# lizhiqi49/threestudio-3dgs

Hardware: AMD Instinct MI355X
Metric: rendered views/sec fwd+bwd @1M Gaussians, 1024², SH=3; 1/2/4/8 GPU (higher is better)
Workload: dtype fp32

## Files before the change

include/gsr.h:

```cpp
#ifndef GSR_H
#define GSR_H

#include <stddef.h>
#include <stdint.h>

#ifdef __cplusplus
extern "C" {
#endif

#define GSR_OK 0
#define GSR_EINVAL 1
#define GSR_EHIP 2

#define GSR_TILE_X 16
#define GSR_TILE_Y 16

const char* gsr_version(void);
#define GSR_ABI_VERSION 9
int gsr_abi_version(void);
const char* gsr_last_error(void);

size_t gsr_geom_bytes(int P);
size_t gsr_binning_bytes(int K, int width, int height);
size_t gsr_image_bytes(int width, int height);
// ... 285 lines not shown
int gsr_sugar_deform_forward(const gsr_sugar_deform* in, float* xyz, float* rot, float* scale, void* stream);
int gsr_sugar_deform_backward(const gsr_sugar_deform* in, const int* sp_order, const int* sp_offsets,
                              const int* col_order, const int* col_offsets, const int* t_order, const int* t_offsets,
                              const float* dL_dxyz, const float* dL_drot, const float* dL_dscale,
                              float* const* dL_dplanes, float* const* dL_dmlp, void* workspace, size_t workspace_bytes,
                              void* stream);

#define GSR_MESHREG_FORWARD 0
#define GSR_MESHREG_NC_BACKWARD 1
#define GSR_MESHREG_LAP_BACKWARD 2
typedef struct gsr_sugar_meshreg {
  int T, V, E, P;
  const float* vert_xyz;
  const int* pairs;
  const int* slot_offsets;
  const int* slots;
  const int* ring_offsets;
  const int* ring;
} gsr_sugar_meshreg;
size_t gsr_sugar_meshreg_workspace_bytes(int T, int V, int P, int pass);
int gsr_sugar_normal_consistency_forward(const gsr_sugar_meshreg* in, float* nc, void* workspace,
                                         size_t workspace_bytes, void* stream);
int gsr_sugar_normal_consistency_backward(const gsr_sugar_meshreg* in, const float* dL_dnc, float* dL_dvert_xyz,
                                          void* workspace, size_t workspace_bytes, void* stream);
int gsr_sugar_laplacian_forward(const gsr_sugar_meshreg* in, float* lap, void* workspace, size_t workspace_bytes,
                                void* stream);
int gsr_sugar_laplacian_backward(const gsr_sugar_meshreg* in, const float* dL_dlap, float* dL_dvert_xyz,
                                 void* workspace, size_t workspace_bytes, void* stream);

size_t gsr_sort_work_bytes(int V, const int* n);
int gsr_sort_pairs(int V, const int* n, uint32_t* keys, uint32_t* vals, int key_bits, int max_bits, void* work,
                   size_t work_bytes, void* stream);
int gsr_sort_rank_mode(void);

int gsr_mark_visible(int P, const float* means3D, const float* viewmatrix, const float* projmatrix,
                     uint8_t* present, void* stream);

#ifdef __cplusplus
}
#endif

#endif
```

threestudio-3dgs_amd/csrc/gsr_api.hip:

```cpp
#include <stdio.h>
#include <string.h>

#include <cmath>
#include <mutex>
#include <vector>

#include "../../include/gsr.h"
#include "gsr_kernels.h"

using namespace gsr;

static thread_local char g_err[512] = "";

static int fail(int code, const char* fmt, const char* what) {
  snprintf(g_err, sizeof(g_err), fmt, what);
  return code;
}

#define GSR_HIP_CHECK(expr)                                                        \
  do {                                                                             \
    hipError_t e_ = (expr);                                                        \
    if (e_ != hipSuccess) return fail(GSR_EHIP, "HIP error: %s", hipGetErrorString(e_)); \
  } while (0)

// ... 213 lines not shown
  hipStream_t s = (hipStream_t)stream;
  GeomState g = GeomState::carve(state->geom, V, P, nullptr);

  PreprocessArgs a;
  a.V = V;
  a.P = P;
  a.deg = effective_degree(sc.degree, sc.M);
  a.M = sc.M;
  a.means3D = sc.means3D;
  a.scales = sc.scales;
  a.rotations = sc.rotations;
  a.opacities = sc.opacities;
  a.shs = sc.shs;
  a.colors_precomp = sc.colors_precomp;
  a.cov3D_precomp = sc.cov3D_precomp;
  a.scale_modifier = sc.scale_modifier;
  a.W = sc.width;
  a.H = sc.height;
  a.radii = state->radii;
  a.col2 = colors2;
  {
    PhaseScope ps(GSR_PHASE_PREPROCESS, s);
    launch_preprocess(a, cams, g, s);
  }
  {
    PhaseScope ps(GSR_PHASE_DEPTH_SORT, s);
    SegInfo seg;
    seg.V = V;
    for (int v = 0; v < V; ++v) {
      seg.n[v] = (uint32_t)P;
      seg.start[v] = (uint32_t)((size_t)v * P);
    }
    seg.rebase = g.drange + 128;
    const int res = seg_sort(g.dkey, g.dval, false, seg, 0, 32, g.sort_counts, g.sort_totals, s);
    if (res != depth_sort_result()) return fail(GSR_EHIP, "%s", "internal: depth sort result buffer");
    launch_binning_counts(V, P, g, s);
  }
  return last_launch();
}

int gsr_composite_forward(int V, int height, int width, const float* color, const float* alpha, const float* bg,
                          int bg_layout, float* out, void* stream) {
  if (V < 0 || height < 0 || width < 0 || bg_layout < 0 || bg_layout > 2) return fail(GSR_EINVAL, "%s", "bad sizes");
  if (V == 0 || height == 0 || width == 0) return last_launch();
  if (color == nullptr || alpha == nullptr || bg == nullptr || out == nullptr)
    return fail(GSR_EINVAL, "%s", "null pointer argument");
  launch_composite_fwd(V, (size_t)height * width, color, alpha, bg, bg_layout, out, (hipStream_t)stream);
  return last_launch();
}

int gsr_composite_backward(int V, int height, int width, const float* dL_dout, const float* color,
                           const float* alpha, const float* bg, int bg_layout, float* dL_dcolor, float* dL_dalpha,
                           float* dL_dbg, void* stream) {
  if (V < 0 || height < 0 || width < 0 || bg_layout < 0 || bg_layout > 2) return fail(GSR_EINVAL, "%s", "bad sizes");
  if (V == 0 || height == 0 || width == 0) return last_launch();
  if (dL_dout == nullptr || color == nullptr || alpha == nullptr || bg == nullptr || dL_dcolor == nullptr ||
      dL_dalpha == nullptr)
    return fail(GSR_EINVAL, "%s", "null pointer argument");
  if (dL_dbg != nullptr && bg_layout == GSR_BG_CONSTANT)
    return fail(GSR_EINVAL, "%s", "dL_dbg is computed for image backgrounds only");
  launch_composite_bwd(V, (size_t)height * width, dL_dout, color, alpha, bg, bg_layout, dL_dcolor, dL_dalpha,
                       dL_dbg, (hipStream_t)stream);
  return last_launch();
}

int gsr_normal_map_forward(int V, int height, int width, const float* normal, const float* alpha, float* out,
                           void* stream) {
// ... 672 lines not shown
  if (!set_total(V, n, seg, &total)) return 0;
  size_t b = 0;
  SortWork::carve(nullptr, V, total, seg.blk[V], &b);
  return b;
}

int gsr_sort_pairs(int V, const int* n, uint32_t* keys, uint32_t* vals, int key_bits, int max_bits, void* work,
                   size_t work_bytes, void* stream) {
  if (V < 1 || V > GSR_SET_MAX) return fail(GSR_EINVAL, "%s", "1..64 segments");
  if (n == nullptr || keys == nullptr || work == nullptr) return fail(GSR_EINVAL, "%s", "null pointer argument");
  if (key_bits < 1 || key_bits > 32 || max_bits < 1 || max_bits > GSR_RADIX_BITS)
    return fail(GSR_EINVAL, "%s", "key_bits must be 1..32 and max_bits 1..8");
  SegInfo seg;
  long long total = 0;
  if (inst_segments(V, n, seg, &total) != GSR_OK) return GSR_EINVAL;
  size_t need = 0;
  SortWork w = SortWork::carve(work, V, total, seg.blk[V], &need);
  if (work_bytes < need) return fail(GSR_EINVAL, "%s", "sort work buffer too small");
  if (total == 0) return last_launch();
  hipStream_t s = (hipStream_t)stream;
  uint32_t* kk[2] = {keys, w.keys2};
  uint32_t* vv[2] = {vals, vals != nullptr ? w.vals2 : nullptr};
  const int r = seg_sort(kk, vals != nullptr ? vv : nullptr, false, seg, 0, key_bits, w.counts, w.totals, s,
                         max_bits);
  if (r == 1) {
    GSR_HIP_CHECK(hipMemcpyAsync(keys, w.keys2, sizeof(uint32_t) * (size_t)total, hipMemcpyDeviceToDevice, s));
    if (vals != nullptr)
      GSR_HIP_CHECK(hipMemcpyAsync(vals, w.vals2, sizeof(uint32_t) * (size_t)total, hipMemcpyDeviceToDevice, s));
  }
  return last_launch();
}

int gsr_sort_rank_mode(void) { return sort_rank_mode(); }

int gsr_set_num_rendered(int V, const void* geom, int P, int* num_rendered, int* num_visible, int* num_listed,
                         void* stream) {
  if (check_set(V, P) != GSR_OK) return GSR_EINVAL;
  if (geom == nullptr || num_rendered == nullptr) return fail(GSR_EINVAL, "%s", "null pointer argument");
  GeomState g = GeomState::carve((void*)geom, V, P, nullptr);
  hipStream_t s = (hipStream_t)stream;
  static thread_local uint32_t* pinned = nullptr;
  if (pinned == nullptr) GSR_HIP_CHECK(hipHostMalloc((void**)&pinned, 3 * GSR_SET_MAX * sizeof(uint32_t), hipHostMallocDefault));
  GSR_HIP_CHECK(hipMemcpyAsync(pinned, g.counters, 3 * (size_t)V * sizeof(uint32_t), hipMemcpyDeviceToHost, s));
  GSR_HIP_CHECK(hipStreamSynchronize(s));
  for (int v = 0; v < V; ++v) {
    num_rendered[v] = (int)pinned[v];
    if (num_visible) num_visible[v] = (int)pinned[V + v];
    if (num_listed) num_listed[v] = (int)pinned[2 * V + v];
    if (pinned[v] > 0x7fffffffu) return fail(GSR_EINVAL, "%s", "instance count of a view exceeds 2^31");
  }
  g_err[0] = 0;
  return GSR_OK;
}

int gsr_set_gauss_state(int V, const void* geom, int P, void* out_rec, void* out_tiles, void* stream) {
  if (check_set(V, P) != GSR_OK) return GSR_EINVAL;
  if (geom == nullptr) return fail(GSR_EINVAL, "%s", "null pointer argument");
  if (P == 0) return GSR_OK;
  GeomState g = GeomState::carve((void*)geom, V, P, nullptr);
  hipStream_t s = (hipStream_t)stream;
  const size_t n = (size_t)V * (size_t)P;
  if (out_rec) GSR_HIP_CHECK(hipMemcpyAsync(out_rec, g.rec, n * sizeof(GaussRec), hipMemcpyDeviceToDevice, s));
  if (out_tiles) GSR_HIP_CHECK(hipMemcpyAsync(out_tiles, g.tiles, n * sizeof(uint2), hipMemcpyDeviceToDevice, s));
  return last_launch();
}

// ... 362 lines not shown
```

threestudio-3dgs_amd/csrc/gsr_common.h:

```cpp
#pragma once

#include <hip/hip_runtime.h>

#if !defined(GSR_DIAG_BUILD) &&                                                                          \
    (defined(GSR_EXP_COALROWS) || defined(GSR_EXP_FWD_NOC) || defined(GSR_EXP_LDSPAD) ||                  \
     defined(GSR_EXP_NOCULL) || defined(GSR_EXP_NOFLUSH) || defined(GSR_EXP_NOGROUP) ||                   \
     defined(GSR_EXP_NOMFMA) || defined(GSR_EXP_NOREACH) || defined(GSR_EXP_NOREPLAY) ||                \
     defined(GSR_EXP_NOCOL2) || defined(GSR_EXP_HOTREC) || defined(GSR_EXP_NOEMBED))
#error "GSR_EXP_* experiment switches build only through `make exp` (a diagnostic library, not libgsr_hip.so)"
#endif
#include <stddef.h>
#include <stdlib.h>
#include <string.h>
#include <stdint.h>

#define GSR_TILE_X 16
#define GSR_TILE_Y 16
#define GSR_TILE_PIX (GSR_TILE_X * GSR_TILE_Y)

#define GSR_SET_MAX 64
#define GSR_SORT_THREADS 256
#ifndef GSR_SORT_ITEMS
#define GSR_SORT_ITEMS 16
#endif
// ... 48 lines not shown
  TilePack t;
  t.tile_bits = tile_key_bits(W, H);
  int gb = 1;
  while (gb < 32 && (1ll << gb) < (long long)P) ++gb;
  t.packed = gb + t.tile_bits <= 32 && !force;
  t.gbits = t.packed ? gb : 0;
  t.gmask = t.packed ? (uint32_t)((1ull << gb) - 1ull) : 0xFFFFFFFFu;
  t.qmask = !t.packed && t.tile_bits <= GSR_QMASK_SHIFT && force_mode != 2;
  t.tmask = t.tile_bits >= 32 ? 0xFFFFFFFFu : (uint32_t)((1ull << t.tile_bits) - 1ull);
  return t;
}

struct DigitPlan {
  int passes, bits;
  __host__ __device__ int width(int p, int key_bits) const {
    const int lo = p * bits;
    return key_bits - lo < bits ? key_bits - lo : bits;
  }
};
static inline DigitPlan digit_plan(int key_bits, int max_bits = GSR_RADIX_BITS) {
  if (key_bits < 1) key_bits = 1;
  if (max_bits < 1 || max_bits > GSR_RADIX_BITS) max_bits = GSR_RADIX_BITS;
  DigitPlan d;
  d.passes = (key_bits + max_bits - 1) / max_bits;
  d.bits = (key_bits + d.passes - 1) / d.passes;
  return d;
}
struct SegInfo {
  int V, tile;
  uint32_t n[GSR_SET_MAX];
  uint32_t start[GSR_SET_MAX];
  uint32_t blk[GSR_SET_MAX + 1];
  const uint32_t* ndev = nullptr;
  const uint32_t* rebase = nullptr;
};
__device__ __forceinline__ uint32_t seg_live(const SegInfo& s, int v) {
  return s.ndev ? min(s.ndev[v], s.n[v]) : s.n[v];
}
__device__ __forceinline__ uint32_t seg_key_base(const SegInfo& s) { return s.rebase ? s.rebase[0] : 0u; }
__device__ __forceinline__ uint32_t seg_key(uint32_t kb, uint32_t key) {
  return key == 0xFFFFFFFFu ? key : key - kb;
}
__device__ __forceinline__ bool seg_skip_last(const SegInfo& s, int last) {
  return last && s.rebase != nullptr && s.rebase[1] != 0u;
}
static inline void seg_fill_blocks(SegInfo& s, int tile) {
  s.tile = tile;
  s.blk[0] = 0;
  for (int v = 0; v < s.V; ++v) s.blk[v + 1] = s.blk[v] + (uint32_t)div_up((long long)s.n[v], tile);
}
__device__ __forceinline__ uint32_t xcd_block(uint32_t b, uint32_t n) {
  const uint32_t x = b & 7u, q = n >> 3, r = n & 7u;
  return x * q + (x < r ? x : r) + (b >> 3);
}
__device__ __forceinline__ int seg_of_block(const SegInfo& s, uint32_t b, uint32_t& lb) {
  int lo = 0, hi = s.V;
  while (hi - lo > 1) {
    const int mid = (lo + hi) >> 1;
    if (s.blk[mid] <= b) lo = mid;
    else hi = mid;
  }
  lb = b - s.blk[lo];
  return lo;
}

struct ViewCam {
  const float *view, *proj, *campos;
  float tanx, tany;
  float fx, fy;
};
struct SetCams {
  ViewCam c[GSR_SET_MAX];
};

struct __attribute__((aligned(64))) GaussRec {
  float4 a, b, c;
  uint4 d;
// ... 10 lines not shown
  uint32_t* goff;
  uint32_t* goff_part;
  uint32_t* vis_part;
  int vbits;
  __host__ __device__ uint32_t vmask() const { return vbits >= 32 ? 0xFFFFFFFFu : (1u << vbits) - 1u; }
  __host__ __device__ uint32_t vsent() const { return vbits > 26 ? 0u : (1u << (32 - vbits)) - 1u; }
  uint32_t* drange;
  __device__ const uint32_t* sorted_dval() const { return drange[129] ? dval[1] : dval[0]; }
  __device__ const uint32_t* sorted_dkey() const { return drange[129] ? dkey[1] : dkey[0]; }
  uint32_t* counters;
  static int sort_blocks(int P) { return div_up(P > 0 ? P : 1, GSR_SORT_TILE); }
  static int dup_blocks(int P) { return div_up(P > 0 ? P : 1, GSR_DUP_TILE); }
  static int goff_blocks(int P) { return div_up(P > 0 ? P : 1, GSR_GOFF_TILE); }
  static GeomState carve(void* base, int V, int P, size_t* bytes) {
    Carver c(base);
    GeomState g;
    const size_t n = (size_t)(V > 0 ? V : 1) * (size_t)(P > 0 ? P : 1);
    const size_t nv = (size_t)(V > 0 ? V : 1);
    g.rec = c.take<GaussRec>(n);
    g.tiles = c.take<uint2>(n);
    g.dkey[0] = c.take<uint32_t>(n);
    g.dkey[1] = c.take<uint32_t>(n);
    g.dval[0] = c.take<uint32_t>(n);
    g.dval[1] = c.take<uint32_t>(n);
    g.sort_counts = c.take<uint32_t>(nv * GSR_RADIX * sort_blocks(P));
    g.sort_totals = c.take<uint32_t>(nv * GSR_RADIX);
    g.kept_counts = c.take<uint32_t>(nv * dup_blocks(P));
    g.counters = c.take<uint32_t>(3 * nv + 64);
    g.goff = c.take<uint32_t>(n);
    g.goff_part = c.take<uint32_t>(nv * goff_blocks(P));
    g.vis_part = c.take<uint32_t>(nv * goff_blocks(P));
    g.vbits = 1;
    while (g.vbits < 32 && (1ull << g.vbits) < (unsigned long long)(P > 1 ? P : 2)) ++g.vbits;
    g.drange = c.take<uint32_t>(132);
    if (bytes) *bytes = align_up(c.off, 256);
    return g;
  }
};

struct BinningState {
  uint32_t* key[2];
  uint32_t* val[2];
  uint32_t* sort_counts;
  uint32_t* sort_totals;
  static BinningState carve(void* base, int V, long long Ktot, long long sort_blocks, bool with_vals, size_t* bytes) {
    Carver c(base);
    BinningState b;
    const size_t n = (size_t)(Ktot > 0 ? Ktot : 1);
    b.key[0] = c.take<uint32_t>(n);
    b.key[1] = c.take<uint32_t>(n);
    b.val[0] = with_vals ? c.take<uint32_t>(n) : nullptr;
    b.val[1] = with_vals ? c.take<uint32_t>(n) : nullptr;
    b.sort_counts = c.take<uint32_t>((size_t)GSR_RADIX * (size_t)(sort_blocks > 0 ? sort_blocks : 1));
    b.sort_totals = c.take<uint32_t>((size_t)GSR_RADIX * (size_t)(V > 0 ? V : 1));
    if (bytes) *bytes = align_up(c.off, 256);
    return b;
  }
};

#define GSR_SPLIT_MAX_TILES 4096
#define GSR_SPLIT_CH 256
#define GSR_SPLIT_NCK 15
__host__ __device__ inline bool split_fits(int V, size_t tiles) {
  return V >= 1 && tiles > 0 && (size_t)V * tiles <= GSR_SPLIT_MAX_TILES;
}
__host__ __device__ inline int split_extra(int V, size_t tiles) {
  const size_t e = (size_t)V * tiles / 4;
// ... 182 lines not shown
```

threestudio-3dgs_amd/csrc/gsr_kernels.h:

```cpp
#pragma once

#include "../../include/gsr.h"
#include "gsr_common.h"

namespace gsr {

int seg_sort(uint32_t* keys[2], uint32_t* vals[2], bool vals_identity, SegInfo seg, int bit_lo, int key_bits,
             uint32_t* counts, uint32_t* totals, hipStream_t stream, int max_bits = GSR_RADIX_BITS);
struct RunWork {
  uint32_t* keys[2];
  uint32_t* vals[2];
  uint32_t *counts, *totals;
  uint32_t* bounds;
  void carve(Carver& c, size_t items, size_t n, float** coef = nullptr) {
    for (int i = 0; i < 2; ++i) keys[i] = c.take<uint32_t>(items);
    for (int i = 0; i < 2; ++i) vals[i] = c.take<uint32_t>(items);
    if (coef) *coef = c.take<float>(items);
    counts = c.take<uint32_t>((size_t)GSR_RADIX * (size_t)div_up((long long)items, GSR_SORT_TILE));
    totals = c.take<uint32_t>((size_t)GSR_RADIX);
    bounds = c.take<uint32_t>(2 * n);
  }
};
int sort_runs(RunWork w, uint32_t n, int N, int* half, hipStream_t stream);
int sort_rank_mode();

struct PreprocessArgs {
  int V, P, deg, M;
  const float *means3D, *scales, *rotations, *opacities, *shs, *colors_precomp, *cov3D_precomp;
  float scale_modifier;
  int W, H;
  int* radii;
  const float* col2;
};
void launch_preprocess(const PreprocessArgs& a, const SetCams& cams, const GeomState& g, hipStream_t stream);

void launch_binning_counts(int V, int P, const GeomState& g, hipStream_t stream);
void launch_emit(int V, int P, int W, const GeomState& g, const SegInfo& inst, const TilePack& tp, uint32_t* keys,
                 uint32_t* vals, hipStream_t stream);
void launch_tile_ranges(SegInfo inst, int n_tiles, const TilePack& tp, const uint32_t* keys, uint2* ranges,
                        hipStream_t stream);
void launch_mark_visible(int P, const float* means3D, const float* view, const float* proj,
                         uint8_t* present, hipStream_t stream);

__device__ __forceinline__ float quad_form(float a, float b, float c, float u, float v) {
  return fmaf(a * u, u, fmaf(2.0f * b * u, v, c * v * v));
}
__device__ __forceinline__ bool quadrant_hit(const float4 r0, const float4 r1, float qx, float qy) {
  const float o = r1.y;
  if (!(o >= GSR_ALPHA_MIN * 0.9999f)) return false;
  const float a = r0.z, b = r0.w, c = r1.x;
  if (!(a > 0.0f && c > 0.0f && a * c - b * b > 0.0f)) return true;
  const float tau = fmaxf(0.0f, __logf(255.0f * o));
  const float thr = 2.0f * (tau * 1.002f + 2e-3f);
  const float u1 = r0.x - qx, u0 = u1 - 7.0f;
  const float v1 = r0.y - qy, v0 = v1 - 7.0f;
  if (u0 <= 0.0f && u1 >= 0.0f && v0 <= 0.0f && v1 >= 0.0f) return true;
  const float ia = 1.0f / a, ic = 1.0f / c;
// ... 180 lines not shown
```

threestudio-3dgs_amd/csrc/gsr_preprocess.hip:

```cpp
#include "gsr_kernels.h"
#include "gsr_math.h"

namespace gsr {

void launch_preprocess_kernel(const PreprocessArgs& a, const SetCams& cams, const GeomState& g, hipStream_t stream);

#ifndef GSR_PRE_VIEWS
#define GSR_PRE_VIEWS 64
#endif
#define GSR_PRE_GAUSS 128
#define GSR_PRE_LDS_FLOATS (8 * 1024)

template <bool SH_LDS>
__attribute__((amdgpu_waves_per_eu(6, 8)))
__global__ __launch_bounds__(256) void k_preprocess(PreprocessArgs a, SetCams cams, GeomState g) {
  extern __shared__ float s_sh[];
  const int nvc = (a.V + GSR_PRE_VIEWS - 1) / GSR_PRE_VIEWS;
  const int vc = blockIdx.x % nvc;
  const int idx0 = (blockIdx.x / nvc) * GSR_PRE_GAUSS;
  const int t = threadIdx.x;
  const int gl = t % GSR_PRE_GAUSS;
  const int half = __builtin_amdgcn_readfirstlane(t / GSR_PRE_GAUSS);
  const int idx = idx0 + gl;
  const int vb = vc * GSR_PRE_VIEWS, ve = min(a.V, vb + GSR_PRE_VIEWS);
// ... 121 lines not shown
    kmn = min(kmn, (uint32_t)__shfl_xor((int)kmn, o, 64));
    kmx = max(kmx, (uint32_t)__shfl_xor((int)kmx, o, 64));
  }
  if ((t & 63) == 0) s_rng[0][t >> 6] = kmn, s_rng[1][t >> 6] = kmx;
  __syncthreads();
  if (t == 0) {
    kmn = min(min(s_rng[0][0], s_rng[0][1]), min(s_rng[0][2], s_rng[0][3]));
    kmx = max(max(s_rng[1][0], s_rng[1][1]), max(s_rng[1][2], s_rng[1][3]));
    if (kmn != 0xFFFFFFFFu) {
      atomicMin(&g.drange[blockIdx.x & 63], kmn);
      atomicMax(&g.drange[64 + (blockIdx.x & 63)], kmx);
    }
  }
}

__global__ void k_depth_range_init(uint32_t* drange, unsigned long long col2) {
  drange[threadIdx.x] = 0xFFFFFFFFu;
  drange[64 + threadIdx.x] = 0u;
  if (threadIdx.x < 2) drange[130 + threadIdx.x] = (uint32_t)(col2 >> (32 * threadIdx.x));
}

__global__ void k_depth_range(uint32_t* drange) {
  const int t = threadIdx.x;
  uint32_t mn = drange[t], mx = drange[64 + t];
#pragma unroll
  for (int o = 32; o > 0; o >>= 1) {
    mn = min(mn, (uint32_t)__shfl_xor((int)mn, o, 64));
    mx = max(mx, (uint32_t)__shfl_xor((int)mx, o, 64));
  }
  if (t == 0) {
    const bool any = mn != 0xFFFFFFFFu;
    drange[128] = any ? mn : 0u;
    drange[129] = (!any || mx - mn < 0x00FFFFFFu) ? 1u : 0u;
  }
}

void launch_preprocess(const PreprocessArgs& a, const SetCams& cams, const GeomState& g, hipStream_t stream) {
  hipLaunchKernelGGL(k_depth_range_init, dim3(1), dim3(64), 0, stream, g.drange,
                     (unsigned long long)(uintptr_t)(a.P > 0 ? a.col2 : nullptr));
  if (a.P > 0 && a.V > 0) launch_preprocess_kernel(a, cams, g, stream);
  hipLaunchKernelGGL(k_depth_range, dim3(1), dim3(64), 0, stream, g.drange);
}

void launch_preprocess_kernel(const PreprocessArgs& a, const SetCams& cams, const GeomState& g, hipStream_t stream) {
  const int nvc = (a.V + GSR_PRE_VIEWS - 1) / GSR_PRE_VIEWS;
  const size_t want = a.colors_precomp == nullptr ? (size_t)GSR_PRE_GAUSS * (3 * a.M + 1) : 0;
  const bool sh_lds = a.colors_precomp == nullptr && a.M > 0 && want <= GSR_PRE_LDS_FLOATS;
  const size_t lds = sh_lds ? sizeof(float) * want : 0;
  hipLaunchKernelGGL(sh_lds ? k_preprocess<true> : k_preprocess<false>,
                     dim3(nvc * ((a.P + GSR_PRE_GAUSS - 1) / GSR_PRE_GAUSS)), dim3(256), lds, stream, a, cams, g);
}

}
```

threestudio-3dgs_amd/csrc/gsr_sort.hip:

```cpp
#include <cstdlib>
#include <cstring>
#include <type_traits>

#include "gsr_kernels.h"
#include "gsr_wave.h"

namespace gsr {

#ifndef GSR_COUNT_SUB
#define GSR_COUNT_SUB 4
#endif
template <int BITS>
__global__ __launch_bounds__(GSR_SORT_THREADS) void k_seg_count(const uint32_t* __restrict__ keys, SegInfo seg,
                                                                int shift, int bits_rt, int last,
                                                                uint32_t* __restrict__ counts) {
  const int bits = BITS ? BITS : bits_rt;
  if (seg_skip_last(seg, last)) return;
  const uint32_t kb = seg_key_base(seg);
  __shared__ uint32_t s_hist[GSR_COUNT_SUB * (GSR_RADIX + 1)];
  const int t = threadIdx.x, lane = t & 63, w = t >> 6;
  uint32_t lb;
  const int v = seg_of_block(seg, xcd_block(blockIdx.x, gridDim.x), lb);
  const uint32_t n = seg_live(seg, v);
  const uint32_t* src = keys + seg.start[v];
  const uint32_t mask = (1u << bits) - 1u;
  const int R = 1 << bits;
  for (int i = t; i < GSR_COUNT_SUB * (GSR_RADIX + 1); i += GSR_SORT_THREADS) s_hist[i] = 0u;
  __syncthreads();
  uint32_t* const hist = s_hist + (lane & (GSR_COUNT_SUB - 1)) * (GSR_RADIX + 1);
  const uint32_t b0 = lb * GSR_SORT_TILE + w * (GSR_SORT_TILE / 4);
  auto body = [&](auto full_c) {
    constexpr bool FULL = decltype(full_c)::value;
    uint32_t key[GSR_SORT_ITEMS];
#pragma unroll
    for (int k = 0; k < GSR_SORT_ITEMS; ++k) {
      const uint32_t i = b0 + k * 64 + lane;
      key[k] = FULL || i < n ? src[i] : 0u;
    }
#pragma unroll
    for (int k = 0; k < GSR_SORT_ITEMS; ++k) {
      const bool valid = FULL || b0 + k * 64 + lane < n;
      const uint32_t d = (seg_key(kb, key[k]) >> shift) & mask;
      if (valid) atomicAdd(&hist[d], 1u);
    }
  };
  if ((lb + 1) * GSR_SORT_TILE <= n)
    body(std::true_type{});
  else
    body(std::false_type{});
  __syncthreads();
  if (t < R) {
    const uint32_t nb = seg.blk[v + 1] - seg.blk[v];
    uint32_t c = 0u;
#pragma unroll
    for (int sb = 0; sb < GSR_COUNT_SUB; ++sb) c += s_hist[sb * (GSR_RADIX + 1) + t];
    counts[(size_t)R * seg.blk[v] + (size_t)t * nb + lb] = c;
  }
}

__global__ __launch_bounds__(256) void k_seg_scan(SegInfo seg, int R, int last, uint32_t* __restrict__ counts,
                                                  uint32_t* __restrict__ totals) {
  if (seg_skip_last(seg, last)) return;
  __shared__ uint32_t s_wave[8];
  const int v = blockIdx.x / R, d = blockIdx.x % R;
  const int t = threadIdx.x;
  const uint32_t nb = seg.blk[v + 1] - seg.blk[v];
  uint32_t* row = counts + (size_t)R * seg.blk[v] + (size_t)d * nb;
  uint32_t carry = 0u;
  for (uint32_t c0 = 0; c0 < nb; c0 += 256 * 4) {
    uint32_t x[4], run = 0u;
#pragma unroll
    for (int k = 0; k < 4; ++k) {
      const uint32_t i = c0 + 4 * t + k;
      const uint32_t c = i < nb ? row[i] : 0u;
      x[k] = run;
      run += c;
    }
    uint32_t tot;
    const uint32_t off = carry + block_exclusive_scan<256>(run, &tot, s_wave);
#pragma unroll
    for (int k = 0; k < 4; ++k) {
      const uint32_t i = c0 + 4 * t + k;
      if (i < nb) row[i] = off + x[k];
    }
    carry += tot;
  }
  if (t == 0) totals[(size_t)v * GSR_RADIX + d] = carry;
}

template <bool KV>
struct ScatterLDS {
  uint32_t keys[GSR_SORT_TILE];
  uint32_t vals[KV ? GSR_SORT_TILE : 1];
  uint32_t wcnt[4][GSR_RADIX];
  uint32_t glob[GSR_RADIX];
  uint32_t wave[8];
};

template <bool KV, int BITS, bool ATOMIC>
__attribute__((amdgpu_waves_per_eu(KV ? 4 : 5, 8)))
__global__ __launch_bounds__(GSR_SORT_THREADS) void k_seg_scatter(
    const uint32_t* __restrict__ keys_in, const uint32_t* __restrict__ vals_in, uint32_t* __restrict__ keys_out,
    uint32_t* __restrict__ vals_out, SegInfo seg, int shift, int bits_rt, int last, const uint32_t* __restrict__ counts,
    const uint32_t* __restrict__ totals) {
  const int bits = BITS ? BITS : bits_rt;
  if (seg_skip_last(seg, last)) return;
  const uint32_t kb = seg_key_base(seg);
  __shared__ ScatterLDS<KV> s;
  const int t = threadIdx.x, lane = t & 63, w = t >> 6;
  uint32_t lb;
  const int v = seg_of_block(seg, xcd_block(blockIdx.x, gridDim.x), lb);
  const uint32_t n = seg_live(seg, v);
  const uint32_t start = seg.start[v];
  const uint32_t mask = (1u << bits) - 1u;
  const int R = 1 << bits;
#pragma unroll
  for (int ww = 0; ww < 4; ++ww) s.wcnt[ww][t] = 0u;
  const uint32_t nb = seg.blk[v + 1] - seg.blk[v];
  const uint32_t dtot = t < R ? totals[(size_t)v * GSR_RADIX + t] : 0u;
  const uint32_t dcnt = t < R ? counts[(size_t)R * seg.blk[v] + (size_t)t * nb + lb] : 0u;
  const uint32_t b0 = lb * GSR_SORT_TILE + w * (GSR_SORT_TILE / 4);
  auto body = [&](auto full_c) {
    constexpr bool FULL = decltype(full_c)::value;
    uint32_t key[GSR_SORT_ITEMS], val[GSR_SORT_ITEMS];
    uint32_t pos2[GSR_SORT_ITEMS / 2];
#pragma unroll
    for (int k = 0; k < GSR_SORT_ITEMS; ++k) {
      const uint32_t i = b0 + k * 64 + lane;
      key[k] = FULL || i < n ? keys_in[start + i] : 0u;
      if (KV) val[k] = FULL || i < n ? (vals_in ? vals_in[start + i] : i) : 0u;
    }
    __syncthreads();
#pragma unroll
    for (int k = 0; k < GSR_SORT_ITEMS; ++k) {
      const bool valid = FULL || b0 + k * 64 + lane < n;
      const uint32_t d = (seg_key(kb, key[k]) >> shift) & mask;
    if (ATOMIC) {
      const uint32_t pk = valid ? atomicAdd(&s.wcnt[w][d], 1u) : 0u;
      pos2[k >> 1] = (k & 1) ? (pos2[k >> 1] | (pk << 16)) : pk;
    } else {
      const unsigned long long peers = match_digit(d, bits, valid);
      const uint32_t rank = mask_rank(peers);
      const uint32_t base = s.wcnt[w][d];
      asm volatile("" ::: "memory");
// ... 72 lines not shown
      case 0: d = (uint32_t)r & 63u; break;
      case 1: d = ((uint32_t)lane >> (r & 7)) & 63u; break;
      case 2: d = ((uint32_t)lane & ((r >> 2) & 7u)) & 63u; break;
      default: d = (h >> 26) & 63u; break;
    }
    const uint32_t got = atomicAdd(&cnt[w][d], 1u);
    const unsigned long long peers = match_digit(d, 6, true);
    const uint32_t first = (uint32_t)__shfl((int)got, (int)__builtin_ctzll(peers), 64);
    err |= (got - first) != mask_rank(peers) ? 1u : 0u;
  }
  if (err) atomicOr(bad, 1u);
}

int sort_rank_mode() {
  static const int mode = [] {
    const char* e = getenv("GSR_SORT_RANK");
    if (e != nullptr && strcmp(e, "ballot") == 0) return 0;
    uint32_t* d = nullptr;
    uint32_t h = 1u;
    if (hipMalloc(&d, sizeof(uint32_t)) != hipSuccess) return 0;
    bool ok = hipMemset(d, 0, sizeof(uint32_t)) == hipSuccess;
    if (ok) {
      hipLaunchKernelGGL(k_lds_rank_probe, dim3(1), dim3(256), 0, 0, d);
      ok = hipGetLastError() == hipSuccess && hipMemcpy(&h, d, sizeof(uint32_t), hipMemcpyDeviceToHost) == hipSuccess;
    }
    (void)hipFree(d);
    return ok && h == 0u ? 1 : 0;
  }();
  return mode;
}
template <int BITS>
static void launch_pass(bool kv, int pass, const uint32_t* kin, const uint32_t* vin, uint32_t* kout, uint32_t* vout,
                        const SegInfo& seg, uint32_t nb, int shift, int bits, int last, uint32_t* counts,
                        uint32_t* totals, hipStream_t stream) {
  hipLaunchKernelGGL(k_seg_count<0>, dim3(nb), dim3(GSR_SORT_THREADS), 0, stream, kin, seg, shift, bits, last,
                     counts);
  hipLaunchKernelGGL(k_seg_scan, dim3(seg.V << bits), dim3(256), 0, stream, seg, 1 << bits, last, counts, totals);
  const int sel = (pass == 0 ? 1 : 2) << (kv ? 2 : 0);
  const bool atomic = (GSR_SORT_ATOMIC_MASK & sel) != 0 && sort_rank_mode() == 1;
  const uint32_t* cc = counts;
  const uint32_t* tt = totals;
  if (kv) {
    if (atomic)
      hipLaunchKernelGGL((k_seg_scatter<true, BITS, true>), dim3(nb), dim3(GSR_SORT_THREADS), 0, stream, kin, vin, kout,
                         vout, seg, shift, bits, last, cc, tt);
    else
      hipLaunchKernelGGL((k_seg_scatter<true, BITS, false>), dim3(nb), dim3(GSR_SORT_THREADS), 0, stream, kin, vin,
                         kout, vout, seg, shift, bits, last, cc, tt);
  } else {
    if (atomic)
      hipLaunchKernelGGL((k_seg_scatter<false, BITS, true>), dim3(nb), dim3(GSR_SORT_THREADS), 0, stream, kin,
                         (const uint32_t*)nullptr, kout, (uint32_t*)nullptr, seg, shift, bits, last, cc, tt);
    else
      hipLaunchKernelGGL((k_seg_scatter<false, BITS, false>), dim3(nb), dim3(GSR_SORT_THREADS), 0, stream, kin,
                         (const uint32_t*)nullptr, kout, (uint32_t*)nullptr, seg, shift, bits, last, cc, tt);
  }
}

int seg_sort(uint32_t* keys[2], uint32_t* vals[2], bool vals_identity, SegInfo seg, int bit_lo, int key_bits,
             uint32_t* counts, uint32_t* totals, hipStream_t stream, int max_bits) {
  const bool kv = vals != nullptr && (vals[0] != nullptr || vals_identity);
  const DigitPlan plan = digit_plan(key_bits, max_bits);
  seg_fill_blocks(seg, GSR_SORT_TILE);
  const uint32_t nb = seg.blk[seg.V];
  int src = 0;
  for (int p = 0; p < plan.passes; ++p) {
    const int bits = plan.width(p, key_bits);
    const int dst = src ^ 1;
    if (nb > 0) {
      const int shift = bit_lo + p * plan.bits;
      const int last = p == plan.passes - 1 ? 1 : 0;
      const uint32_t* vin = (p == 0 && vals_identity) ? nullptr : (kv ? vals[src] : nullptr);
      uint32_t* vout = kv ? vals[dst] : nullptr;
      if (bits == 8)
        launch_pass<8>(kv, p, keys[src], vin, keys[dst], vout, seg, nb, shift, bits, last, counts, totals, stream);
      else if (bits == 6)
        launch_pass<6>(kv, p, keys[src], vin, keys[dst], vout, seg, nb, shift, bits, last, counts, totals, stream);
      else if (bits == 4)
        launch_pass<4>(kv, p, keys[src], vin, keys[dst], vout, seg, nb, shift, bits, last, counts, totals, stream);
      else
        launch_pass<0>(kv, p, keys[src], vin, keys[dst], vout, seg, nb, shift, bits, last, counts, totals, stream);
    }
    src = dst;
  }
  return src;
}

__global__ __launch_bounds__(256) void k_run_bounds(const uint32_t* __restrict__ keys, uint32_t n, uint32_t N,
                                                    uint32_t* __restrict__ begin, uint32_t* __restrict__ end) {
  const long long i = (long long)blockIdx.x * 256 + threadIdx.x;
  if (i >= (long long)n) return;
  const uint32_t key = keys[i];
  if (key >= N) return;
  if (i == 0 || keys[i - 1] != key) begin[key] = (uint32_t)i;
  if (i + 1 == (long long)n || keys[i + 1] != key) end[key] = (uint32_t)i + 1u;
}

int sort_runs(RunWork w, uint32_t n, int N, int* half, hipStream_t stream) {
  hipError_t err = hipMemsetAsync(w.bounds, 0, sizeof(uint32_t) * 2 * (size_t)N, stream);
  if (err != hipSuccess) return (int)err;
  SegInfo seg{};
  seg.V = 1;
  seg.n[0] = n;
  seg.start[0] = 0u;
  int key_bits = 1;
  while (key_bits < 32 && (1ull << key_bits) <= (unsigned long long)N) ++key_bits;
  *half = seg_sort(w.keys, w.vals, true, seg, 0, key_bits, w.counts, w.totals, stream);
  hipLaunchKernelGGL(k_run_bounds, dim3(div_up((long long)n, 256)), dim3(256), 0, stream, w.keys[*half], n,
                     (uint32_t)N, w.bounds, w.bounds + N);
  return 0;
}

}
```

threestudio-3dgs_amd/diff_gaussian_rasterization/_C.py:

```python
from __future__ import annotations

import collections
import ctypes
import os

import torch

_HERE = os.path.dirname(os.path.abspath(__file__))
LIB_PATH = os.environ.get("GSR_HIP_LIB", os.path.join(_HERE, "libgsr_hip.so"))

_lib = None

_vp = ctypes.c_void_p
_i = ctypes.c_int
_f = ctypes.c_float
_sz = ctypes.c_size_t
_P = ctypes.POINTER
_ip, _fp, _vpp = _P(_i), _P(_f), _P(_vp)


def _fields(ctype, names):
    return [(n, ctype) for n in names.split()]


# ... 69 lines not shown
SIGNATURES = {
    "gsr_version": (ctypes.c_char_p, []),
    "gsr_abi_version": (_i, []),
    "gsr_last_error": (ctypes.c_char_p, []),
    "gsr_geom_bytes": (_sz, [_i]),
    "gsr_binning_bytes": (_sz, [_i, _i, _i]),
    "gsr_image_bytes": (_sz, [_i, _i]),
    "gsr_backward_bytes": (_sz, [_i, _i]),
    "gsr_forward_preprocess": (
        _i,
        [_i, _i, _i, _vp, _vp, _f, _vp, _vp, _vp, _vp, _vp, _vp, _vp, _vp, _i, _i, _f, _f, _i, _vp, _vp, _vp],
    ),
    "gsr_num_rendered": (_i, [_vp, _i, ctypes.POINTER(_i), ctypes.POINTER(_i), _vp]),
    "gsr_forward_render": (_i, [_i, _i, _i, _i, _vp, _vp, _vp, _vp, _vp, _vp, _vp, _vp]),
    "gsr_backward": (
        _i,
        [_i, _i, _i, _i, _i, _i, _vp, _vp, _vp, _f, _vp, _vp, _vp, _vp, _vp, _vp, _vp, _vp, _f, _f,
         _vp, _vp, _vp, _vp, _vp, _vp, _vp, _vp, _vp, _vp, _vp, _vp, _vp, _vp, _vp, _vp, _vp],
    ),
    "gsr_mark_visible": (_i, [_i, _vp, _vp, _vp, _vp, _vp]),
    "gsr_composite_forward": (_i, [_i, _i, _i, _vp, _vp, _vp, _i, _vp, _vp]),
    "gsr_composite_backward": (_i, [_i, _i, _i, _vp, _vp, _vp, _vp, _i, _vp, _vp, _vp, _vp]),
    "gsr_normal_map_forward": (_i, [_i, _i, _i, _vp, _vp, _vp, _vp]),
    "gsr_normal_map_backward": (_i, [_i, _i, _i, _vp, _vp, _vp, _vp, _vp, _vp]),
    "gsr_shade_forward": (_i, [_i, _i, _i, _i, _i] + [_vp] * 6 + [_i] + [_vp] * 8 + [_vp]),
    "gsr_shade_backward": (_i, [_i, _i, _i, _i, _i] + [_vp] * 6 + [_i] + [_vp] * 12 + [_vp]),
    "gsr_shade_views_forward": (_i, [_i, _i, _i, _i, ctypes.POINTER(_i)] + [_vp] * 6 + [_i] + [_vp] * 2
                                + [ctypes.POINTER(_f)] * 2 + [_vp] * 4 + [_vp]),
    "gsr_shade_views_backward": (_i, [_i, _i, _i, _i, ctypes.POINTER(_i)] + [_vp] * 6 + [_i] + [_vp] * 2
                                 + [ctypes.POINTER(_f)] * 2 + [_vp] * 8 + [_vp]),
    "gsr_sort_work_bytes": (_sz, [_i, ctypes.POINTER(_i)]),
    "gsr_sort_pairs": (_i, [_i, ctypes.POINTER(_i), _vp, _vp, _i, _i, _vp, _sz, _vp]),
    "gsr_sort_rank_mode": (_i, []),
    "gsr_knn_workspace_bytes": (_sz, [_i]),
    "gsr_knn_mean_dist": (_i, [_i, _vp, _vp, _vp, _sz, _vp]),
    "gsr_knn_points_workspace_bytes": (_sz, [_i, _i]),
    "gsr_knn_points": (_i, [_i, _i, _vp, _vp, _vp, _vp, _sz, _vp]),
    "gsr_sugar_field_workspace_bytes": (_sz, [_i, _i, _i]),
    "gsr_sugar_field_forward": (_i, [_P(SugarField)] + [_vp] * 3 + [_vp, _sz, _vp]),
    "gsr_sugar_field_backward": (_i, [_P(SugarField)] + [_vp] * 3 + [_vp] * 5 + [_vp, _sz, _vp]),
    "gsr_sugar_normal_workspace_bytes": (_sz, [_i, _i, _i]),
    "gsr_sugar_normal_forward": (_i, [_P(SugarNormal)] + [_vp] * 2 + [_vp, _sz, _vp]),
    "gsr_sugar_normal_backward": (_i, [_P(SugarNormal)] + [_vp] * 2 + [_vp] + [_vp, _sz, _vp]),
    "gsr_sugar_mesh_workspace_bytes": (_sz, [_i, _i]),
    "gsr_sugar_mesh_forward": (_i, [_P(SugarMesh), _i, _vp, _f] + [_vp] * 4 + [_vp]),
    "gsr_sugar_mesh_backward": (_i, [_P(SugarMesh), _i, _vp] + [_vp] * 2 + [_vp] * 4 + [_vp] * 3 + [_vp, _sz, _vp]),
    "gsr_sugar_skin_workspace_bytes": (_sz, [_i, _i, _i]),
    "gsr_sugar_skin_forward": (_i, [_P(SugarSkin)] + [_vp] * 3 + [_vp, _sz, _vp]),
    "gsr_sugar_skin_backward": (_i, [_P(SugarSkin)] + [_vp] * 2 + [_vp] * 3 + [_vp] * 4 + [_vp, _sz, _vp]),
    "gsr_sugar_timed_workspace_bytes": (_sz, [_i, _i]),
    "gsr_sugar_timed_forward": (_i, [_P(SugarTimed), _i, _vp] + [_vp] * 4 + [_vp]),
    "gsr_sugar_timed_backward": (_i, [_P(SugarTimed), _i, _vp] + [_vp] * 2 + [_vp] * 4 + [_vp] * 5 + [_vp, _sz, _vp]),
    "gsr_sugar_arap_workspace_bytes": (_sz, [_i, _i]),
    "gsr_sugar_arap_forward": (_i, [_P(SugarArap)] + [_vp] + [_vp, _sz, _vp]),
    "gsr_sugar_arap_backward": (_i, [_P(SugarArap)] + [_vp] + [_vp] * 2 + [_vp]),
    "gsr_sugar_spline_workspace_bytes": (_sz, [_i, _i, _i]),
    "gsr_sugar_spline_forward": (_i, [_P(SugarSpline)] + [_vp] * 3 + [_vp]),
    "gsr_sugar_spline_backward": (_i, [_P(SugarSpline)] + [_vp] * 3 + [_vp] * 3 + [_vp, _sz, _vp]),
    "gsr_sugar_deform_workspace_bytes": (_sz, [_i, _i, _i]),
    "gsr_sugar_deform_forward": (_i, [_P(SugarDeform)] + [_vp] * 3 + [_vp]),
    "gsr_sugar_deform_backward": (_i, [_P(SugarDeform)] + [_vp] * 6 + [_vp] * 3 + [_vpp] * 2 + [_vp, _sz, _vp]),
    "gsr_sugar_meshreg_workspace_bytes": (_sz, [_i, _i, _i, _i]),
    "gsr_sugar_normal_consistency_forward": (_i, [_P(SugarMeshReg)] + [_vp] + [_vp, _sz, _vp]),
    "gsr_sugar_normal_consistency_backward": (_i, [_P(SugarMeshReg)] + [_vp] + [_vp] + [_vp, _sz, _vp]),
    "gsr_sugar_laplacian_forward": (_i, [_P(SugarMeshReg)] + [_vp] + [_vp, _sz, _vp]),
    "gsr_sugar_laplacian_backward": (_i, [_P(SugarMeshReg)] + [_vp] + [_vp] + [_vp, _sz, _vp]),
# ... 273 lines not shown
```

Baseline: 3994.

## Replace LSD depth sort with MSD pass plus per-bucket LDS finish

The per-view depth sort becomes a hybrid. First one most-significant-digit radix pass runs on the rebased depth key, with a dynamic shift sized to the depth span. Then a single-block kernel sorts each bucket in LDS, provided every bucket fits under a cap. Views whose buckets overflow, or whose span is too wide, fall back to the existing multi-pass LSD sort through per-view gate flags. The aim is to replace several global scatter passes over about 1M keys per view with one global pass and local work, at the cost of added gating complexity and a fallback path for skewed depth distributions.

```diff
diff --git a/include/gsr.h b/include/gsr.h
--- a/include/gsr.h
+++ b/include/gsr.h
@@ -341,6 +341,9 @@
 int gsr_sort_pairs(int V, const int* n, uint32_t* keys, uint32_t* vals, int key_bits, int max_bits, void* work,
                    size_t work_bytes, void* stream);
 int gsr_sort_rank_mode(void);
+size_t gsr_sort_depth_work_bytes(int V, const int* n);
+int gsr_sort_pairs_depth(int V, const int* n, uint32_t* keys, uint32_t* vals, uint32_t rebase_base, uint32_t span,
+                         int cap_pairs, int* lsd_views, void* work, size_t work_bytes, void* stream);
 
 int gsr_mark_visible(int P, const float* means3D, const float* viewmatrix, const float* projmatrix,
                      uint8_t* present, void* stream);
diff --git a/threestudio-3dgs_amd/csrc/gsr_api.hip b/threestudio-3dgs_amd/csrc/gsr_api.hip
--- a/threestudio-3dgs_amd/csrc/gsr_api.hip
+++ b/threestudio-3dgs_amd/csrc/gsr_api.hip
@@ -269,7 +269,7 @@
       seg.start[v] = (uint32_t)((size_t)v * P);
     }
     seg.rebase = g.drange + 128;
-    const int res = seg_sort(g.dkey, g.dval, false, seg, 0, 32, g.sort_counts, g.sort_totals, s);
+    const int res = depth_sort(g.dkey, g.dval, seg, g.sort_counts, g.sort_totals, 0u, s);
     if (res != depth_sort_result()) return fail(GSR_EHIP, "%s", "internal: depth sort result buffer");
     launch_binning_counts(V, P, g, s);
   }
@@ -1008,6 +1008,52 @@
 }
 
 int gsr_sort_rank_mode(void) { return sort_rank_mode(); }
+
+static size_t sort_depth_plan_offset(size_t sort_bytes) { return align_up(sort_bytes, 256); }
+size_t gsr_sort_depth_work_bytes(int V, const int* n) {
+  const size_t b = gsr_sort_work_bytes(V, n);
+  return b == 0 ? 0 : sort_depth_plan_offset(b) + align_up(sizeof(uint32_t) * GSR_REBASE_WORDS, 256);
+}
+
+int gsr_sort_pairs_depth(int V, const int* n, uint32_t* keys, uint32_t* vals, uint32_t rebase_base, uint32_t span,
+                         int cap_pairs, int* lsd_views, void* work, size_t work_bytes, void* stream) {
+  if (V < 1 || V > GSR_SET_MAX) return fail(GSR_EINVAL, "%s", "1..64 segments");
+  if (n == nullptr || keys == nullptr || vals == nullptr || work == nullptr)
+    return fail(GSR_EINVAL, "%s", "null pointer argument");
+  if (cap_pairs < 0 || cap_pairs > GSR_MSD_CAP) return fail(GSR_EINVAL, "%s", "cap_pairs must be 0..GSR_MSD_CAP");
+  SegInfo seg;
+  long long total = 0;
+  if (inst_segments(V, n, seg, &total) != GSR_OK) return GSR_EINVAL;
+  size_t sort_bytes = 0;
+  SortWork w = SortWork::carve(work, V, total, seg.blk[V], &sort_bytes);
+  if (work_bytes < gsr_sort_depth_work_bytes(V, n)) return fail(GSR_EINVAL, "%s", "sort work buffer too small");
+  hipStream_t s = (hipStream_t)stream;
+  uint32_t* plan = (uint32_t*)((char*)work + sort_depth_plan_offset(sort_bytes));
+  const bool fits = span < 0x00FFFFFFu;
+  uint32_t host[GSR_REBASE_WORDS] = {};
+  host[0] = rebase_base;
+  host[1] = fits ? 1u : 0u;
+  host[GSR_MSD_SHIFT] = msd_shift(span);
+  GSR_HIP_CHECK(hipMemcpyAsync(plan, host, sizeof(host), hipMemcpyHostToDevice, s));
+  GSR_HIP_CHECK(hipStreamSynchronize(s));
+  if (total > 0) {
+    seg.rebase = plan;
+    uint32_t* kk[2] = {keys, w.keys2};
+    uint32_t* vv[2] = {vals, w.vals2};
+    const int r = depth_sort(kk, vv, seg, w.counts, w.totals, (uint32_t)cap_pairs, s);
+    if (r != 0) return fail(GSR_EHIP, "%s", "internal: depth sort result buffer");
+    if (fits) {
+      GSR_HIP_CHECK(hipMemcpyAsync(keys, w.keys2, sizeof(uint32_t) * (size_t)total, hipMemcpyDeviceToDevice, s));
+      GSR_HIP_CHECK(hipMemcpyAsync(vals, w.vals2, sizeof(uint32_t) * (size_t)total, hipMemcpyDeviceToDevice, s));
+    }
+  }
+  if (lsd_views != nullptr) {
+    GSR_HIP_CHECK(hipMemcpyAsync(host, plan, sizeof(host), hipMemcpyDeviceToHost, s));
+    GSR_HIP_CHECK(hipStreamSynchronize(s));
+    for (int v = 0; v < V; ++v) lsd_views[v] = !depth_sort_msd() || host[GSR_MSD_FLAG + v] != 0u ? 1 : 0;
+  }
+  return last_launch();
+}
 
 int gsr_set_num_rendered(int V, const void* geom, int P, int* num_rendered, int* num_visible, int* num_listed,
                          void* stream) {
diff --git a/threestudio-3dgs_amd/csrc/gsr_common.h b/threestudio-3dgs_amd/csrc/gsr_common.h
--- a/threestudio-3dgs_amd/csrc/gsr_common.h
+++ b/threestudio-3dgs_amd/csrc/gsr_common.h
@@ -104,7 +104,26 @@
   uint32_t start[GSR_SET_MAX];
   uint32_t blk[GSR_SET_MAX + 1];
   const uint32_t* ndev = nullptr;
-  const uint32_t* rebase = nullptr;
+  uint32_t* rebase = nullptr;
+};
+#define GSR_MSD_THREADS 512
+#define GSR_MSD_ITEMS 16
+#define GSR_MSD_CAP (GSR_MSD_THREADS * GSR_MSD_ITEMS)
+#define GSR_MSD_SHIFT 4
+#define GSR_MSD_FLAG 8
+#define GSR_REBASE_WORDS (GSR_MSD_FLAG + GSR_SET_MAX)
+__host__ __device__ static inline uint32_t msd_shift(uint32_t span) {
+  uint32_t s = 0u;
+  while ((span >> s) >= 255u) ++s;
+  return s;
+}
+enum SegGate {
+  GSR_GATE_ALL = 0,
+  GSR_GATE_LAST = 1,
+  GSR_GATE_MSD_PLAN = 2,
+  GSR_GATE_MSD = 3,
+  GSR_GATE_LSD = 4,
+  GSR_GATE_LSD_LAST = 5,
 };
 __device__ __forceinline__ uint32_t seg_live(const SegInfo& s, int v) {
   return s.ndev ? min(s.ndev[v], s.n[v]) : s.n[v];
@@ -113,8 +132,16 @@
 __device__ __forceinline__ uint32_t seg_key(uint32_t kb, uint32_t key) {
   return key == 0xFFFFFFFFu ? key : key - kb;
 }
-__device__ __forceinline__ bool seg_skip_last(const SegInfo& s, int last) {
-  return last && s.rebase != nullptr && s.rebase[1] != 0u;
+__device__ __forceinline__ bool seg_skip_all(const SegInfo& s, int gate) {
+  return (gate == GSR_GATE_LAST || gate == GSR_GATE_LSD_LAST) && s.rebase != nullptr && s.rebase[1] != 0u;
+}
+__device__ __forceinline__ bool seg_skip_view(const SegInfo& s, int gate, int v) {
+  if (gate < GSR_GATE_MSD) return false;
+  const bool lsd = s.rebase[GSR_MSD_FLAG + v] != 0u;
+  return gate == GSR_GATE_MSD ? lsd : !lsd;
+}
+__device__ __forceinline__ int seg_shift(const SegInfo& s, int shift) {
+  return shift < 0 ? (int)s.rebase[GSR_MSD_SHIFT] : shift;
 }
 static inline void seg_fill_blocks(SegInfo& s, int tile) {
   s.tile = tile;
@@ -191,7 +218,7 @@
     g.vis_part = c.take<uint32_t>(nv * goff_blocks(P));
     g.vbits = 1;
     while (g.vbits < 32 && (1ull << g.vbits) < (unsigned long long)(P > 1 ? P : 2)) ++g.vbits;
-    g.drange = c.take<uint32_t>(132);
+    g.drange = c.take<uint32_t>(128 + GSR_REBASE_WORDS);
     if (bytes) *bytes = align_up(c.off, 256);
     return g;
   }
diff --git a/threestudio-3dgs_amd/csrc/gsr_kernels.h b/threestudio-3dgs_amd/csrc/gsr_kernels.h
--- a/threestudio-3dgs_amd/csrc/gsr_kernels.h
+++ b/threestudio-3dgs_amd/csrc/gsr_kernels.h
@@ -23,6 +23,9 @@
 };
 int sort_runs(RunWork w, uint32_t n, int N, int* half, hipStream_t stream);
 int sort_rank_mode();
+int depth_sort(uint32_t* keys[2], uint32_t* vals[2], SegInfo seg, uint32_t* counts, uint32_t* totals, uint32_t cap,
+               hipStream_t stream);
+int depth_sort_msd();
 
 struct PreprocessArgs {
   int V, P, deg, M;
diff --git a/threestudio-3dgs_amd/csrc/gsr_preprocess.hip b/threestudio-3dgs_amd/csrc/gsr_preprocess.hip
--- a/threestudio-3dgs_amd/csrc/gsr_preprocess.hip
+++ b/threestudio-3dgs_amd/csrc/gsr_preprocess.hip
@@ -177,6 +177,7 @@
     const bool any = mn != 0xFFFFFFFFu;
     drange[128] = any ? mn : 0u;
     drange[129] = (!any || mx - mn < 0x00FFFFFFu) ? 1u : 0u;
+    drange[128 + GSR_MSD_SHIFT] = any ? msd_shift(mx - mn) : 0u;
   }
 }
 
diff --git a/threestudio-3dgs_amd/csrc/gsr_sort.hip b/threestudio-3dgs_amd/csrc/gsr_sort.hip
--- a/threestudio-3dgs_amd/csrc/gsr_sort.hip
+++ b/threestudio-3dgs_amd/csrc/gsr_sort.hip
@@ -12,15 +12,22 @@
 #endif
 template <int BITS>
 __global__ __launch_bounds__(GSR_SORT_THREADS) void k_seg_count(const uint32_t* __restrict__ keys, SegInfo seg,
-                                                                int shift, int bits_rt, int last,
+                                                                int shift_h, int bits_rt, int gate,
                                                                 uint32_t* __restrict__ counts) {
   const int bits = BITS ? BITS : bits_rt;
-  if (seg_skip_last(seg, last)) return;
+  if (seg_skip_all(seg, gate)) return;
   const uint32_t kb = seg_key_base(seg);
+  const int shift = seg_shift(seg, shift_h);
   __shared__ uint32_t s_hist[GSR_COUNT_SUB * (GSR_RADIX + 1)];
   const int t = threadIdx.x, lane = t & 63, w = t >> 6;
   uint32_t lb;
   const int v = seg_of_block(seg, xcd_block(blockIdx.x, gridDim.x), lb);
+  if (gate == GSR_GATE_MSD_PLAN) {
+    const bool wide = seg.rebase[1] == 0u;
+    if (lb == 0u && t == 0) seg.rebase[GSR_MSD_FLAG + v] = wide ? 1u : 0u;
+    if (wide) return;
+  }
+  if (seg_skip_view(seg, gate, v)) return;
   const uint32_t n = seg_live(seg, v);
   const uint32_t* src = keys + seg.start[v];
   const uint32_t mask = (1u << bits) - 1u;
@@ -58,11 +65,13 @@
   }
 }
 
-__global__ __launch_bounds__(256) void k_seg_scan(SegInfo seg, int R, int last, uint32_t* __restrict__ counts,
-                                                  uint32_t* __restrict__ totals) {
-  if (seg_skip_last(seg, last)) return;
+__global__ __launch_bounds__(256) void k_seg_scan(SegInfo seg, int R, int gate, uint32_t cap,
+                                                  uint32_t* __restrict__ counts, uint32_t* __restrict__ totals) {
+  if (seg_skip_all(seg, gate)) return;
+  if (gate == GSR_GATE_MSD_PLAN && seg.rebase[1] == 0u) return;
   __shared__ uint32_t s_wave[8];
   const int v = blockIdx.x / R, d = blockIdx.x % R;
+  if (seg_skip_view(seg, gate, v)) return;
   const int t = threadIdx.x;
   const uint32_t nb = seg.blk[v + 1] - seg.blk[v];
   uint32_t* row = counts + (size_t)R * seg.blk[v] + (size_t)d * nb;
@@ -85,7 +94,10 @@
     }
     carry += tot;
   }
-  if (t == 0) totals[(size_t)v * GSR_RADIX + d] = carry;
+  if (t == 0) {
+    totals[(size_t)v * GSR_RADIX + d] = carry;
+    if (gate == GSR_GATE_MSD_PLAN && d < GSR_RADIX - 1 && carry > cap) atomicOr(&seg.rebase[GSR_MSD_FLAG + v], 1u);
+  }
 }
 
 template <bool KV>
@@ -101,15 +113,17 @@
 __attribute__((amdgpu_waves_per_eu(KV ? 4 : 5, 8)))
 __global__ __launch_bounds__(GSR_SORT_THREADS) void k_seg_scatter(
     const uint32_t* __restrict__ keys_in, const uint32_t* __restrict__ vals_in, uint32_t* __restrict__ keys_out,
-    uint32_t* __restrict__ vals_out, SegInfo seg, int shift, int bits_rt, int last, const uint32_t* __restrict__ counts,
-    const uint32_t* __restrict__ totals) {
+    uint32_t* __restrict__ vals_out, SegInfo seg, int shift_h, int bits_rt, int gate,
+    const uint32_t* __restrict__ counts, const uint32_t* __restrict__ totals) {
   const int bits = BITS ? BITS : bits_rt;
-  if (seg_skip_last(seg, last)) return;
+  if (seg_skip_all(seg, gate)) return;
   const uint32_t kb = seg_key_base(seg);
+  const int shift = seg_shift(seg, shift_h);
   __shared__ ScatterLDS<KV> s;
   const int t = threadIdx.x, lane = t & 63, w = t >> 6;
   uint32_t lb;
   const int v = seg_of_block(seg, xcd_block(blockIdx.x, gridDim.x), lb);
+  if (seg_skip_view(seg, gate, v)) return;
   const uint32_t n = seg_live(seg, v);
   const uint32_t start = seg.start[v];
   const uint32_t mask = (1u << bits) - 1u;
@@ -248,10 +262,12 @@
 template <int BITS>
 static void launch_pass(bool kv, int pass, const uint32_t* kin, const uint32_t* vin, uint32_t* kout, uint32_t* vout,
                         const SegInfo& seg, uint32_t nb, int shift, int bits, int last, uint32_t* counts,
-                        uint32_t* totals, hipStream_t stream) {
+                        uint32_t* totals, hipStream_t stream, uint32_t cap = 0u) {
   hipLaunchKernelGGL(k_seg_count<0>, dim3(nb), dim3(GSR_SORT_THREADS), 0, stream, kin, seg, shift, bits, last,
                      counts);
-  hipLaunchKernelGGL(k_seg_scan, dim3(seg.V << bits), dim3(256), 0, stream, seg, 1 << bits, last, counts, totals);
+  hipLaunchKernelGGL(k_seg_scan, dim3(seg.V << bits), dim3(256), 0, stream, seg, 1 << bits, last, cap, counts,
+                     totals);
+  if (last == GSR_GATE_MSD_PLAN) last = GSR_GATE_MSD;
   const int sel = (pass == 0 ? 1 : 2) << (kv ? 2 : 0);
   const bool atomic = (GSR_SORT_ATOMIC_MASK & sel) != 0 && sort_rank_mode() == 1;
   const uint32_t* cc = counts;
@@ -273,8 +289,18 @@
   }
 }
 
+static int seg_sort_gated(uint32_t* keys[2], uint32_t* vals[2], bool vals_identity, SegInfo seg, int bit_lo,
+                          int key_bits, uint32_t* counts, uint32_t* totals, hipStream_t stream, int max_bits, int gate,
+                          int gate_last);
+
 int seg_sort(uint32_t* keys[2], uint32_t* vals[2], bool vals_identity, SegInfo seg, int bit_lo, int key_bits,
              uint32_t* counts, uint32_t* totals, hipStream_t stream, int max_bits) {
+  return seg_sort_gated(keys, vals, vals_identity, seg, bit_lo, key_bits, counts, totals, stream, max_bits,
+                        GSR_GATE_ALL, seg.rebase != nullptr ? GSR_GATE_LAST : GSR_GATE_ALL);
+}
+
+static int seg_sort_gated(uint32_t* keys[2], uint32_t* vals[2], bool vals_identity, SegInfo seg, int bit_lo, int key_bits,
+                   uint32_t* counts, uint32_t* totals, hipStream_t stream, int max_bits, int gate, int gate_last) {
   const bool kv = vals != nullptr && (vals[0] != nullptr || vals_identity);
   const DigitPlan plan = digit_plan(key_bits, max_bits);
   seg_fill_blocks(seg, GSR_SORT_TILE);
@@ -285,7 +311,7 @@
     const int dst = src ^ 1;
     if (nb > 0) {
       const int shift = bit_lo + p * plan.bits;
-      const int last = p == plan.passes - 1 ? 1 : 0;
+      const int last = p == plan.passes - 1 ? gate_last : gate;
       const uint32_t* vin = (p == 0 && vals_identity) ? nullptr : (kv ? vals[src] : nullptr);
       uint32_t* vout = kv ? vals[dst] : nullptr;
       if (bits == 8)
@@ -300,6 +326,130 @@
     src = dst;
   }
   return src;
+}
+
+struct FinishLDS {
+  uint32_t keys[GSR_MSD_CAP];
+  uint32_t vals[GSR_MSD_CAP];
+  uint32_t wcnt[GSR_MSD_THREADS / 64][GSR_RADIX];
+  uint32_t wave[GSR_MSD_THREADS / 64 + 1];
+};
+
+__global__ __launch_bounds__(GSR_MSD_THREADS) void k_msd_finish(uint32_t* __restrict__ keys,
+                                                                uint32_t* __restrict__ vals, SegInfo seg,
+                                                                const uint32_t* __restrict__ totals) {
+  constexpr int NW = GSR_MSD_THREADS / 64;
+  __shared__ FinishLDS s;
+  const int t = threadIdx.x, lane = t & 63, w = t >> 6;
+  const int v = blockIdx.x / (GSR_RADIX - 1), d = blockIdx.x % (GSR_RADIX - 1);
+  if (seg.rebase[GSR_MSD_FLAG + v] != 0u) return;
+  const int shift = (int)seg.rebase[GSR_MSD_SHIFT];
+  const uint32_t kb = seg.rebase[0];
+  const uint32_t n = totals[(size_t)v * GSR_RADIX + d];
+  if (n <= 1u || n > (uint32_t)GSR_MSD_CAP || shift == 0) return;
+  const uint32_t before = block_sum_u32<GSR_MSD_THREADS>(t < d ? totals[(size_t)v * GSR_RADIX + t] : 0u, s.wave);
+  uint32_t* const kp = keys + seg.start[v] + before;
+  uint32_t* const vp = vals + seg.start[v] + before;
+  const uint32_t per = (n + NW * 64 - 1) / (NW * 64) * 64;
+  const uint32_t b0 = (uint32_t)w * per;
+  uint32_t key[GSR_MSD_ITEMS], val[GSR_MSD_ITEMS];
+  uint32_t pos2[GSR_MSD_ITEMS / 2];
+#pragma unroll
+  for (int k = 0; k < GSR_MSD_ITEMS; ++k) {
+    const uint32_t i = b0 + k * 64 + lane;
+    const bool valid = (uint32_t)k * 64u < per && i < n;
+    key[k] = valid ? kp[i] : 0u;
+    val[k] = valid ? vp[i] : 0u;
+  }
+  const int npass = (shift + 7) >> 3;
+  for (int p = 0; p < npass; ++p) {
+    const int sh = 8 * p;
+    for (int i = t; i < NW * GSR_RADIX; i += GSR_MSD_THREADS) (&s.wcnt[0][0])[i] = 0u;
+    if (p > 0) {
+#pragma unroll
+      for (int k = 0; k < GSR_MSD_ITEMS; ++k) {
+        const uint32_t i = b0 + k * 64 + lane;
+        const bool valid = (uint32_t)k * 64u < per && i < n;
+        key[k] = valid ? s.keys[i] : 0u;
+        val[k] = valid ? s.vals[i] : 0u;
+      }
+    }
+    __syncthreads();
+#pragma unroll
+    for (int k = 0; k < GSR_MSD_ITEMS; ++k) {
+      if ((uint32_t)k * 64u < per) {
+        const bool valid = b0 + k * 64 + lane < n;
+        const uint32_t dg = ((key[k] - kb) >> sh) & 255u;
+        const unsigned long long peers = match_digit(dg, 8, valid);
+        const uint32_t rank = mask_rank(peers);
+        const uint32_t base = s.wcnt[w][dg];
+        asm volatile("" ::: "memory");
+        if (valid && rank == 0) s.wcnt[w][dg] = base + (uint32_t)__popcll(peers);
+        const uint32_t pk = base + rank;
+        pos2[k >> 1] = (k & 1) ? (pos2[k >> 1] | (pk << 16)) : pk;
+      } else if (!(k & 1)) {
+        pos2[k >> 1] = 0u;
+      }
+    }
+    __syncthreads();
+    uint32_t wc[NW], bc = 0u;
+    if (t < GSR_RADIX) {
+#pragma unroll
+      for (int ww = 0; ww < NW; ++ww) {
+        wc[ww] = s.wcnt[ww][t];
+        bc += wc[ww];
+      }
+    }
+    uint32_t tot;
+    const uint32_t lstart = block_exclusive_scan<GSR_MSD_THREADS>(bc, &tot, s.wave);
+    if (t < GSR_RADIX) {
+      uint32_t run = lstart;
+#pragma unroll
+      for (int ww = 0; ww < NW; ++ww) {
+        s.wcnt[ww][t] = run;
+        run += wc[ww];
+      }
+    }
+    __syncthreads();
+#pragma unroll
+    for (int k = 0; k < GSR_MSD_ITEMS; ++k) {
+      if ((uint32_t)k * 64u < per && b0 + k * 64 + lane < n) {
+        const uint32_t dg = ((key[k] - kb) >> sh) & 255u;
+        const uint32_t lp = s.wcnt[w][dg] + ((pos2[k >> 1] >> (16 * (k & 1))) & 0xFFFFu);
+        s.keys[lp] = key[k];
+        s.vals[lp] = val[k];
+      }
+    }
+    __syncthreads();
+  }
+  for (uint32_t j = t; j < n; j += GSR_MSD_THREADS) {
+    kp[j] = s.keys[j];
+    vp[j] = s.vals[j];
+  }
+}
+
+int depth_sort_msd() {
+  static const int on = [] {
+    const char* e = getenv("GSR_DEPTH_SORT");
+    return e != nullptr && strcmp(e, "lsd") == 0 ? 0 : 1;
+  }();
+  return on;
+}
+
+int depth_sort(uint32_t* keys[2], uint32_t* vals[2], SegInfo seg, uint32_t* counts, uint32_t* totals, uint32_t cap,
+               hipStream_t stream) {
+  if (!depth_sort_msd()) return seg_sort(keys, vals, false, seg, 0, 32, counts, totals, stream);
+  if (cap == 0u || cap > (uint32_t)GSR_MSD_CAP) cap = GSR_MSD_CAP;
+  seg_fill_blocks(seg, GSR_SORT_TILE);
+  const uint32_t nb = seg.blk[seg.V];
+  if (nb > 0) {
+    launch_pass<8>(true, 0, keys[0], vals[0], keys[1], vals[1], seg, nb, -1, 8, GSR_GATE_MSD_PLAN, counts, totals,
+                   stream, cap);
+    hipLaunchKernelGGL(k_msd_finish, dim3(seg.V * (GSR_RADIX - 1)), dim3(GSR_MSD_THREADS), 0, stream, keys[1], vals[1],
+                       seg, (const uint32_t*)totals);
+  }
+  return seg_sort_gated(keys, vals, false, seg, 0, 32, counts, totals, stream, GSR_RADIX_BITS, GSR_GATE_LSD,
+                        GSR_GATE_LSD_LAST);
 }
 
 __global__ __launch_bounds__(256) void k_run_bounds(const uint32_t* __restrict__ keys, uint32_t n, uint32_t N,
diff --git a/threestudio-3dgs_amd/diff_gaussian_rasterization/_C.py b/threestudio-3dgs_amd/diff_gaussian_rasterization/_C.py
--- a/threestudio-3dgs_amd/diff_gaussian_rasterization/_C.py
+++ b/threestudio-3dgs_amd/diff_gaussian_rasterization/_C.py
@@ -125,6 +125,9 @@
     "gsr_sort_work_bytes": (_sz, [_i, ctypes.POINTER(_i)]),
     "gsr_sort_pairs": (_i, [_i, ctypes.POINTER(_i), _vp, _vp, _i, _i, _vp, _sz, _vp]),
     "gsr_sort_rank_mode": (_i, []),
+    "gsr_sort_depth_work_bytes": (_sz, [_i, ctypes.POINTER(_i)]),
+    "gsr_sort_pairs_depth": (_i, [_i, ctypes.POINTER(_i), _vp, _vp, ctypes.c_uint32, ctypes.c_uint32, _i,
+                                  ctypes.POINTER(_i), _vp, _sz, _vp]),
     "gsr_knn_workspace_bytes": (_sz, [_i]),
     "gsr_knn_mean_dist": (_i, [_i, _vp, _vp, _vp, _sz, _vp]),
     "gsr_knn_points_workspace_bytes": (_sz, [_i, _i]),
```

New measurement: 4003, median of 6. Within noise of the previous version (+0.2%).
